# lswzjuer/pytorch-quantity

Hardware: AMD Instinct MI355X
Metric: calibration images/sec + int8-sim images/sec, ResNet-50 224², 1/2/4/8 GPU (higher is better)
Workload: dtype f32

## Files before the change

### pytorch-quantity_amd/csrc/fq_conv1x1_f32.hip

```cpp
#include "fq_common.h"
#include "fq_producer_stat.h"

#include <utility>

namespace fq {
namespace {

constexpr int kT = 256;
constexpr int kBK = 16;
constexpr int kStepWide = 8;
template <int WM> constexpr int step_of() { return WM == 2 ? kStepWide : kBK; }
typedef float f4v __attribute__((ext_vector_type(4)));
typedef float f16v __attribute__((ext_vector_type(16)));

struct C1Args {
    const float* x;
    const float* wt;
    const unsigned short* wsb;
    const float* bias;
    float* y;
    float* relu;
    const float* res;
    float* sum;
    int store_y;
// ... 1 lines not shown
    int Hin, R, S, pad;
    unsigned x_bytes, w_bytes, y_bytes;
    unsigned cols;
    unsigned tiles_m, tiles;
    int stream_stores;
    unsigned split_first, split_s, work;
    float* ws;
    unsigned* ws_count;
#ifdef FQ_C1_ABLATE
    int ablate;
#endif
};

#ifdef FQ_C1_ABLATE
#define FQ_C1_OFF(bit) (a.ablate & (bit))
#else
#define FQ_C1_OFF(bit) false
#endif

struct NoStat {
    __device__ __forceinline__ void add(float) {}
};

template <typename SC, typename SS, bool kStores>
struct AddStat {
    static constexpr bool kMayStore = kStores;
    SC c;
    SS s;
};
template <typename T> struct is_add_stat { static constexpr bool value = false; };
template <typename SC, typename SS, bool K> struct is_add_stat<AddStat<SC, SS, K>> { static constexpr bool value = true; };

template <int I>
struct Stage {
    static constexpr int value = I;
};

template <int WM, int WN, int BK = kBK>
struct Shape {
    static constexpr int BM = 64 * WM, BN = 64 * WN;
    static constexpr int kXRows = BK * BN / kT;
    static constexpr int kXStep = kT / BN > 0 ? kT / BN : 1;
    static constexpr int kWVecs = BK * BM / 4 / kT;
    static constexpr int kWRowStep = kT / (BM / 4);
    static constexpr int kFloats = 3 * BK * (BM + BN) + BM;
    static_assert(kXRows >= 1 && kWVecs >= 1 && BK % 4 == 0, "tile too small for 256 loading threads");
};

template <int WM, int WN, bool kRelu, bool kStream, bool kFullM, typename Stat>
__device__ __forceinline__ void c1_epilogue(const f16v (&acc)[WM][WN], const C1Args& a, Stat& stat, const float* s_bias,
                                            unsigned jbase, unsigned mbase, unsigned m0, unsigned n0, unsigned r, unsigned h) {
    const __amdgpu_buffer_rsrc_t yrs = __builtin_amdgcn_make_buffer_rsrc(a.y ? a.y : a.relu, 0, a.y ? a.y_bytes : 0u, 0x00020000);
    const __amdgpu_buffer_rsrc_t rrs = __builtin_amdgcn_make_buffer_rsrc(kRelu ? a.relu : a.y, 0, a.y_bytes, 0x00020000);
    constexpr int aux = kStream ? 2 : 0;
#pragma unroll
    for (int ni = 0; ni < WN; ++ni) {
        const unsigned jn = jbase + n0 + 32u * ni + r;
        if (jn < a.cols) {
            const unsigned n = jn / a.HWout, p = jn - n * a.HWout;
            const unsigned col4 = (n * a.Cout * a.HWout + p + (mbase + m0 + 4u * h) * a.HWout) * 4u;
#pragma unroll
            for (int mi = 0; mi < WM; ++mi) {
                f4v b4[4];
#pragma unroll
                for (int q = 0; q < 4; ++q) b4[q] = *reinterpret_cast<const f4v*>(s_bias + m0 + 32u * mi + 8u * q + 4u * h);
#pragma unroll
                for (int e = 0; e < 16; ++e) {
                    const unsigned dm = 32u * mi + (e & 3) + 8u * (e >> 2);
                    if (kFullM || mbase + m0 + 4u * h + dm < a.Cout) {
                        const float val = stat_map(stat, acc[mi][ni][e] + b4[e >> 2][e & 3]);
                        const int row4 = (int)(dm * a.HWout * 4u);
                        __builtin_amdgcn_raw_buffer_store_b32(__builtin_bit_cast(unsigned, val), yrs, (int)col4, row4, aux);
                        if (kRelu)
                            __builtin_amdgcn_raw_buffer_store_b32(__builtin_bit_cast(unsigned, relu_like_torch(val)), rrs, (int)col4,
                                                                  row4, aux);
                        stat.add(val);
                    }
                }
            }
        }
    }
}

template <int WM, int WN, bool kStoreY, bool kStoreSum, bool kStream, typename Stat>
__device__ __forceinline__ void c1_epilogue_add(const f16v (&acc)[WM][WN], const C1Args& a, Stat& stat, const float* s_bias,
                                                unsigned jbase, unsigned mbase, unsigned m0, unsigned n0, unsigned r, unsigned h) {
    const __amdgpu_buffer_rsrc_t yrs = __builtin_amdgcn_make_buffer_rsrc(kStoreY ? a.y : a.relu, 0, a.y_bytes, 0x00020000);
    const __amdgpu_buffer_rsrc_t srs = __builtin_amdgcn_make_buffer_rsrc(kStoreSum ? a.sum : a.relu, 0, a.y_bytes, 0x00020000);
    const __amdgpu_buffer_rsrc_t rrs = __builtin_amdgcn_make_buffer_rsrc(a.relu, 0, a.y_bytes, 0x00020000);
    const __amdgpu_buffer_rsrc_t ers = __builtin_amdgcn_make_buffer_rsrc(const_cast<float*>(a.res), 0, a.y_bytes, 0x00020000);
    constexpr int aux = kStream ? 2 : 0;
#pragma unroll
    for (int ni = 0; ni < WN; ++ni) {
        const unsigned jn = jbase + n0 + 32u * ni + r;
        if (jn < a.cols) {
            const unsigned n = jn / a.HWout, p = jn - n * a.HWout;
            const unsigned col4 = (n * a.Cout * a.HWout + p + (mbase + m0 + 4u * h) * a.HWout) * 4u;
#pragma unroll
            for (int mi = 0; mi < WM; ++mi) {
                float rv[16];
#pragma unroll
                for (int e = 0; e < 16; ++e) {
                    const unsigned dm = 32u * mi + (e & 3) + 8u * (e >> 2);
                    rv[e] = __builtin_bit_cast(float, __builtin_amdgcn_raw_buffer_load_b32(ers, (int)col4, (int)(dm * a.HWout * 4u), aux));
                }
                f4v b4[4];
#pragma unroll
                for (int q = 0; q < 4; ++q) b4[q] = *reinterpret_cast<const f4v*>(s_bias + m0 + 32u * mi + 8u * q + 4u * h);
#pragma unroll
                for (int e = 0; e < 16; ++e) {
                    const unsigned dm = 32u * mi + (e & 3) + 8u * (e >> 2);
                    const int row4 = (int)(dm * a.HWout * 4u);
                    const float val = acc[mi][ni][e] + b4[e >> 2][e & 3];
                    stat.c.add(val);
                    if (kStoreY) __builtin_amdgcn_raw_buffer_store_b32(__builtin_bit_cast(unsigned, val), yrs, (int)col4, row4, aux);
                    const float sm = val + rv[e];
                    stat.s.add(sm);
                    if (kStoreSum) __builtin_amdgcn_raw_buffer_store_b32(__builtin_bit_cast(unsigned, sm), srs, (int)col4, row4, aux);
                    __builtin_amdgcn_raw_buffer_store_b32(__builtin_bit_cast(unsigned, relu_like_torch(sm)), rrs, (int)col4, row4, aux);
                }
            }
        }
    }
}

template <int WM, int WN, typename Stat>
__device__ __forceinline__ void finish_tile(f16v (&acc)[WM][WN], const C1Args& a, Stat& stat, const float* s_bias, bool split, unsigned t,
                                            unsigned slice, unsigned jbase, unsigned mbase, unsigned m0, unsigned n0, unsigned r, unsigned h,
                                            unsigned tid, unsigned wave) {
    constexpr int BM = 64 * WM, BN = 64 * WN;
    bool finish = true;
    if (split) {
        const unsigned rr = t - a.split_first;
        constexpr unsigned kTileFloats = (unsigned)(BM * BN);
        float* const mine = a.ws + ((size_t)rr * a.split_s + slice) * kTileFloats;
#pragma unroll
        for (int mi = 0; mi < WM; ++mi)
#pragma unroll
            for (int ni = 0; ni < WN; ++ni)
#pragma unroll
                for (int q = 0; q < 4; ++q) {
                    const f4v v = {acc[mi][ni][4 * q], acc[mi][ni][4 * q + 1], acc[mi][ni][4 * q + 2], acc[mi][ni][4 * q + 3]};
                    *reinterpret_cast<f4v*>(mine + ((((mi * WN + ni) * 4 + q) * kT) + tid) * 4u) = v;
                }
        asm volatile("s_waitcnt vmcnt(0)" ::: "memory");
        __syncthreads();
        __shared__ unsigned s_last;
        if (tid == 0) {
            __builtin_amdgcn_fence(__ATOMIC_RELEASE, "agent");
            asm volatile("s_waitcnt vmcnt(0)" ::: "memory");
            const unsigned prev = __hip_atomic_fetch_add(a.ws_count + rr, 1u, __ATOMIC_RELAXED, __HIP_MEMORY_SCOPE_AGENT);
            const unsigned last = prev + 1u == a.split_s;
            if (last) {
                __builtin_amdgcn_fence(__ATOMIC_ACQUIRE, "agent");
                asm volatile("s_waitcnt vmcnt(0)" ::: "memory");
                __hip_atomic_store(a.ws_count + rr, 0u, __ATOMIC_RELAXED, __HIP_MEMORY_SCOPE_AGENT);
            }
            s_last = last;
        }
        __syncthreads();
        finish = s_last != 0u;
        if (finish) {
            if (wave != 0) {
                __builtin_amdgcn_fence(__ATOMIC_ACQUIRE, "agent");
                asm volatile("s_waitcnt vmcnt(0)" ::: "memory");
            }
#pragma unroll
            for (int mi = 0; mi < WM; ++mi)
#pragma unroll
                for (int ni = 0; ni < WN; ++ni)
#pragma unroll
                    for (int e = 0; e < 16; ++e) acc[mi][ni][e] = 0.0f;
            for (unsigned sl = 0; sl < a.split_s; ++sl) {
                const float* part = a.ws + ((size_t)rr * a.split_s + sl) * kTileFloats;
#pragma unroll
                for (int mi = 0; mi < WM; ++mi)
#pragma unroll
                    for (int ni = 0; ni < WN; ++ni)
#pragma unroll
                        for (int q = 0; q < 4; ++q) {
                            const f4v v = *reinterpret_cast<const f4v*>(part + ((((mi * WN + ni) * 4 + q) * kT) + tid) * 4u);
#pragma unroll
                            for (int c = 0; c < 4; ++c) acc[mi][ni][4 * q + c] += v[c];
                        }
            }
        }
    }
    if (finish) {
        const bool full_m = mbase + BM <= a.Cout;
#ifdef FQ_C1_ABLATE
        if (FQ_C1_OFF(1)) {
        } else
#endif
#define FQ_C1_EPI(R, S, F) c1_epilogue<WM, WN, R, S, F>(acc, a, stat, s_bias, jbase, mbase, m0, n0, r, h)
#define FQ_C1_ADD(Y, S, N) c1_epilogue_add<WM, WN, Y, S, N>(acc, a, stat, s_bias, jbase, mbase, m0, n0, r, h)
        if constexpr (is_add_stat<Stat>::value) {
            if constexpr (!Stat::kMayStore) {
                if (a.stream_stores) FQ_C1_ADD(false, false, true); else FQ_C1_ADD(false, false, false);
            } else
            if (a.stream_stores) {
                if (a.store_y) { if (a.sum) FQ_C1_ADD(true, true, true); else FQ_C1_ADD(true, false, true); }
                else { if (a.sum) FQ_C1_ADD(false, true, true); else FQ_C1_ADD(false, false, true); }
            } else {
                if (a.store_y) { if (a.sum) FQ_C1_ADD(true, true, false); else FQ_C1_ADD(true, false, false); }
                else { if (a.sum) FQ_C1_ADD(false, true, false); else FQ_C1_ADD(false, false, false); }
            }
// ... 661 lines not shown
    a.Cin = (unsigned)Cin; a.Cout = (unsigned)Cout; a.HWin = (unsigned)(Hin * Win); a.HWout = (unsigned)(Hout * Wout);
    a.Win = (unsigned)Win; a.Wout = (unsigned)Wout; a.stride = (unsigned)stride;
    a.Hin = Hin; a.R = R; a.S = S; a.pad = pad;
    a.cols = (unsigned)cols;
    a.x_bytes = (unsigned)(in_elems * 4);
    a.w_bytes = wsb ? (unsigned)(w_elems * 6) : (unsigned)(w_elems * 4);
    a.y_bytes = (unsigned)(out_elems * 4);
    a.tiles_m = a.tiles = 0;
    a.split_first = a.split_s = a.work = 0; a.ws = nullptr; a.ws_count = nullptr;
    a.stream_stores = out_elems * (relu_out && y ? 8 : 4) > ((size_t)256 << 20);
#ifdef FQ_C1_ABLATE
    a.ablate = env_int("FQ_C1_ABLATE", 0);
#endif
    hipStream_t st = as_stream(stream);
    static const int hist_per_cu = env_int("FQ_CONV1X1_HIST_WG_PER_CU", 0);
    static const int fast = [] { const char* e = getenv("FQ_HIST_IEEE_DIV"); return (e && e[0] && e[0] != '0') ? 0 : 1; }();
    const int mode = taps ? 2 : ((Cin % kBK) != 0 ? 1 : 0);
    static const int forced = env_int("FQ_CONV1X1_SHAPE", 0);
    const size_t tiles22 = ((cols + 127) / 128) * (size_t)((Cout + 127) / 128);
    const int shape = forced ? forced : ((Cout <= 64 || tiles22 <= (size_t)kCUs * 4) ? 12 : 22);
    if (wsb) {
        if (shape == 12) return launch_sb<1, 2>(a, max_inout, interval, hist_row, fast, qd, nullptr, nullptr, nullptr, nullptr, nullptr, nullptr, false, workspace, workspace_bytes, st);
        return launch_sb<2, 2>(a, max_inout, interval, hist_row, fast, qd, nullptr, nullptr, nullptr, nullptr, nullptr, nullptr, false, workspace, workspace_bytes, st);
    }
#define FQ_C1_LAUNCH(WM, WN)                                                                                       \
    do {                                                                                                           \
        if (mode == 2) launch<WM, WN, 2>(a, a.cols, max_inout, interval, hist_row, hist_per_cu, fast, qd, workspace, workspace_bytes, st);     \
        else if (mode == 1) launch<WM, WN, 1>(a, a.cols, max_inout, interval, hist_row, hist_per_cu, fast, qd, workspace, workspace_bytes, st); \
        else launch<WM, WN, 0>(a, a.cols, max_inout, interval, hist_row, hist_per_cu, fast, qd, workspace, workspace_bytes, st);               \
    } while (0)
    if (shape == 12) FQ_C1_LAUNCH(1, 2);
    else FQ_C1_LAUNCH(2, 2);
#undef FQ_C1_LAUNCH
    FQ_LAUNCH_CHECK();
    return FQ_OK;
}

}

extern "C" size_t fq_conv_f32_workspace_bytes(void) { return kSplitWsBytes; }

extern "C" int fq_conv1x1_f32(const float* x, const float* wt, const float* bias, float* y, float* relu_out, int N, int Cin,
                              int Hin, int Win, int Cout, int stride, float* max_inout, const float* interval,
                              int64_t* hist_row, void* workspace, size_t workspace_bytes, fq_stream_t stream) {
    return conv_f32_launch(x, wt, bias, y, relu_out, N, Cin, Hin, Win, Cout, 1, 1, stride, 0, max_inout, interval, hist_row,
                           workspace, workspace_bytes, stream);
}

extern "C" int fq_conv_kxk_f32(const float* x, const float* wt, const float* bias, float* y, float* relu_out, int N, int Cin,
                               int Hin, int Win, int Cout, int R, int S, int stride, int pad, float* max_inout,
                               const float* interval, int64_t* hist_row, void* workspace, size_t workspace_bytes,
                               fq_stream_t stream) {
    return conv_f32_launch(x, wt, bias, y, relu_out, N, Cin, Hin, Win, Cout, R, S, stride, pad, max_inout, interval, hist_row,
                           workspace, workspace_bytes, stream);
}

static int conv_add_launch(const float* x, const float* wt_in, const unsigned short* wsb, const float* bias, const float* res, float* y, float* sum,
                           float* relu_out, int N, int Cin, int Hin, int Win, int Cout, int stride, float* max_y, float* max_sum,
                           const float* interval_y, int64_t* hist_y, const float* interval_sum, int64_t* hist_sum,
                           void* workspace, size_t workspace_bytes, fq_stream_t stream) {
    const float* wt = wsb ? reinterpret_cast<const float*>(wsb) : wt_in;
    if (N < 0 || Cin <= 0 || Hin <= 0 || Win <= 0 || Cout <= 0 || stride < 1) return FQ_ERR_INVALID_ARG;
    if (N == 0) return FQ_OK;
    const bool hist = hist_y != nullptr;
    if (!x || !wt || !res || !relu_out) return FQ_ERR_INVALID_ARG;
    if (hist ? (!hist_sum || !interval_y || !interval_sum || hist_y == hist_sum) : (!max_y || !max_sum)) return FQ_ERR_INVALID_ARG;
    if ((Cin % kBK) != 0 || (Cout % 128) != 0 || (reinterpret_cast<uintptr_t>(wt) & 15u)) return FQ_ERR_UNSUPPORTED;
    const int Hout = (Hin - 1) / stride + 1, Wout = (Win - 1) / stride + 1;
    const size_t cols = (size_t)N * Hout * Wout;
    const size_t in_elems = (size_t)N * Cin * Hin * Win, out_elems = cols * Cout, w_elems = (size_t)Cin * Cout;
    if (cols >= 0xffffff00ULL || in_elems >= (1ULL << 30) || w_elems >= (1ULL << 30) || out_elems >= (1ULL << 30))
        return FQ_ERR_UNSUPPORTED;
    C1Args a;
    a.x = x; a.wt = wt; a.wsb = wsb; a.bias = bias; a.y = y; a.relu = relu_out; a.res = res; a.sum = sum; a.store_y = y != nullptr;
    a.Cin = (unsigned)Cin; a.Cout = (unsigned)Cout; a.HWin = (unsigned)(Hin * Win); a.HWout = (unsigned)(Hout * Wout);
    a.Win = (unsigned)Win; a.Wout = (unsigned)Wout; a.stride = (unsigned)stride;
    a.Hin = Hin; a.R = 1; a.S = 1; a.pad = 0;
    a.cols = (unsigned)cols;
    a.x_bytes = (unsigned)(in_elems * 4); a.w_bytes = wsb ? (unsigned)(w_elems * 6) : (unsigned)(w_elems * 4); a.y_bytes = (unsigned)(out_elems * 4);
    a.stream_stores = out_elems * (size_t)(8 + (y ? 4 : 0) + (sum ? 4 : 0)) > ((size_t)256 << 20) && (a.HWout % 16u) == 0;
    static const int stream_env = env_int("FQ_CONV_ADD_STREAM", -1);
    if (stream_env >= 0) a.stream_stores = stream_env;
#ifdef FQ_C1_ABLATE
    a.ablate = 0;
#endif
    static const int forced = env_int("FQ_CONV1X1_SHAPE", 0);
    const size_t tiles22 = ((cols + 127) / 128) * (size_t)(Cout / 128);
    const bool narrow = forced ? forced == 12 : tiles22 <= (size_t)kCUs * 4;
    hipStream_t st = as_stream(stream);
    a.tiles_m = (unsigned)Cout / (narrow ? 64u : 128u);
    a.tiles = (unsigned)((cols + 127) / 128) * a.tiles_m;
    if (wsb) {
        static const int fast_sb = [] { const char* e = getenv("FQ_HIST_IEEE_DIV"); return (e && e[0] && e[0] != '0') ? 0 : 1; }();
        if (narrow) return launch_sb<1, 2>(a, nullptr, nullptr, nullptr, fast_sb, nullptr, interval_y, hist_y, interval_sum, hist_sum, max_y, max_sum, true, workspace, workspace_bytes, st);
        return launch_sb<2, 2>(a, nullptr, nullptr, nullptr, fast_sb, nullptr, interval_y, hist_y, interval_sum, hist_sum, max_y, max_sum, true, workspace, workspace_bytes, st);
    }
    plan_split(a, (unsigned)Cin / (unsigned)(narrow ? step_of<1>() : step_of<2>()), workspace, workspace_bytes);
    if (hist) {
        static const int fast = [] { const char* e = getenv("FQ_HIST_IEEE_DIV"); return (e && e[0] && e[0] != '0') ? 0 : 1; }();
        static const int res12 = [] {
            int n = 0;
            if (hipOccupancyMaxActiveBlocksPerMultiprocessor(&n, conv1x1_f32_add_hist_kernel<1, 2>, kT, 0) != hipSuccess || n < 1) n = 1;
            return n;
        }();
        static const int res22 = [] {
            int n = 0;
            if (hipOccupancyMaxActiveBlocksPerMultiprocessor(&n, conv1x1_f32_add_hist_kernel<2, 2>, kT, 0) != hipSuccess || n < 1) n = 1;
            return n;
        }();
        unsigned grid = (unsigned)kCUs * (unsigned)(narrow ? res12 : res22);
        if (grid > a.work) grid = a.work;
        unsigned long long* hy = reinterpret_cast<unsigned long long*>(hist_y);
        unsigned long long* hs = reinterpret_cast<unsigned long long*>(hist_sum);
        if (narrow)
            hipLaunchKernelGGL((conv1x1_f32_add_hist_kernel<1, 2>), dim3(grid), dim3(kT), 0, st, a, interval_y, hy, interval_sum, hs, fast);
        else
            hipLaunchKernelGGL((conv1x1_f32_add_hist_kernel<2, 2>), dim3(grid), dim3(kT), 0, st, a, interval_y, hy, interval_sum, hs, fast);
    } else if (narrow) {
        hipLaunchKernelGGL((conv1x1_f32_add_absmax_kernel<1, 2>), dim3(a.work), dim3(kT), 0, st, a,
                           reinterpret_cast<unsigned int*>(max_y), reinterpret_cast<unsigned int*>(max_sum));
    } else {
        hipLaunchKernelGGL((conv1x1_f32_add_absmax_kernel<2, 2>), dim3(a.work), dim3(kT), 0, st, a,
                           reinterpret_cast<unsigned int*>(max_y), reinterpret_cast<unsigned int*>(max_sum));
    }
    FQ_LAUNCH_CHECK();
    return FQ_OK;
}

extern "C" int fq_conv1x1_add_f32(const float* x, const float* wt, const float* bias, const float* res, float* y, float* sum,
                                  float* relu_out, int N, int Cin, int Hin, int Win, int Cout, int stride, float* max_y,
                                  float* max_sum, void* workspace, size_t workspace_bytes, fq_stream_t stream) {
    return conv_add_launch(x, wt, nullptr, bias, res, y, sum, relu_out, N, Cin, Hin, Win, Cout, stride, max_y, max_sum, nullptr, nullptr,
                           nullptr, nullptr, workspace, workspace_bytes, stream);
}

extern "C" int fq_conv1x1_add_hist_f32(const float* x, const float* wt, const float* bias, const float* res, float* relu_out,
                                       int N, int Cin, int Hin, int Win, int Cout, int stride, const float* interval_y,
                                       int64_t* hist_y, const float* interval_sum, int64_t* hist_sum, void* workspace,
                                       size_t workspace_bytes, fq_stream_t stream) {
    if (!hist_y) return FQ_ERR_INVALID_ARG;
    return conv_add_launch(x, wt, nullptr, bias, res, nullptr, nullptr, relu_out, N, Cin, Hin, Win, Cout, stride, nullptr, nullptr, interval_y,
                           hist_y, interval_sum, hist_sum, workspace, workspace_bytes, stream);
}

static bool qd_params(int bit, int bitwidth, QdStat* qd) {
    if ((bitwidth != 8 && bitwidth != 16) || bit < -120 || bit > 120) return false;
    qd->scale = ldexpf(1.0f, bit); qd->inv = ldexpf(1.0f, -bit);
    qd->lo = bitwidth == 8 ? -128.0f : -32768.0f; qd->hi = bitwidth == 8 ? 127.0f : 32767.0f;
    return true;
}

extern "C" int fq_conv1x1_qd_f32(const float* x, const float* wt, const float* bias, float* y, int N, int Cin, int Hin, int Win,
                                 int Cout, int stride, int bit, int bitwidth, void* workspace, size_t workspace_bytes,
                                 fq_stream_t stream) {
    QdStat qd;
    if (!qd_params(bit, bitwidth, &qd)) return FQ_ERR_INVALID_ARG;
    return conv_f32_launch(x, wt, bias, y, nullptr, N, Cin, Hin, Win, Cout, 1, 1, stride, 0, nullptr, nullptr, nullptr, workspace,
                           workspace_bytes, stream, &qd);
}

extern "C" int fq_conv_kxk_qd_f32(const float* x, const float* wt, const float* bias, float* y, int N, int Cin, int Hin, int Win,
                                  int Cout, int R, int S, int stride, int pad, int bit, int bitwidth, void* workspace,
                                  size_t workspace_bytes, fq_stream_t stream) {
    QdStat qd;
    if (!qd_params(bit, bitwidth, &qd)) return FQ_ERR_INVALID_ARG;
    return conv_f32_launch(x, wt, bias, y, nullptr, N, Cin, Hin, Win, Cout, R, S, stride, pad, nullptr, nullptr, nullptr, workspace,
                           workspace_bytes, stream, &qd);
// ... 50 lines not shown
```

### pytorch-quantity_amd/csrc/fq_conv_wino_f32.hip

```cpp
#include "fq_common.h"
#include "fq_producer_stat.h"

#ifndef FQ_WINO_ABLATE
#define FQ_WINO_ABLATE 0
#endif
#define FQ_WINO_OFF(bit) ((FQ_WINO_ABLATE) & (bit))

namespace fq {
namespace {

constexpr unsigned kBK = 64;
constexpr unsigned kCS = 8;
template <int WT>
struct Geo {
    static constexpr int kT = 256 * WT;
    static constexpr unsigned kWaves = 4u * WT;
    static constexpr unsigned kBT = 32u * WT;
    static constexpr unsigned kKkBytes = kBT * 16u;
    static constexpr unsigned kPlane = 2u * kKkBytes;
    static constexpr unsigned kStageBytes = 16u * kPlane;
    static constexpr unsigned kLdsBytes = 3u * kStageBytes;
};
constexpr unsigned kOob = 0x80000000u;
typedef float f2v __attribute__((ext_vector_type(2)));
typedef float f4v __attribute__((ext_vector_type(4)));
typedef float f16v __attribute__((ext_vector_type(16)));
typedef unsigned u2v __attribute__((__vector_size__(2 * sizeof(unsigned))));

struct WArgs {
    const float* x;
    const float* u;
    const float* bias;
    float* y;
    float* relu;
    unsigned Cin, Cout, H, W, HW, TH, TW, tiles_img, tiles, tiles_t, work;
    unsigned x_bytes, u_bytes, y_bytes;
    int stream_stores;
};

struct NoStat {
    __device__ __forceinline__ void add(float) {}
};

__device__ __forceinline__ void stat_add_if(NoStat&, bool, float) {}
__device__ __forceinline__ void stat_add_if(QdStat&, bool, float) {}
__device__ __forceinline__ void stat_add_if(MaxStat& s, bool ok, float v) { s.add(ok ? v : 0.0f); }
template <bool kFast>
__device__ __forceinline__ void stat_add_if(HistStat<kFast>& s, bool ok, float v) { if (ok) s.add(v); }

template <int WT, bool kEven, bool kRelu, bool kStream, typename Stat>
__device__ __forceinline__ void wino_epilogue(const f16v (&acc)[8], unsigned ph, unsigned wave, unsigned lane, char* smem, const WArgs& a,
                                              Stat& stat, unsigned kbase, unsigned tbase, unsigned r, unsigned h) {
    const __amdgpu_buffer_rsrc_t yrs = __builtin_amdgcn_make_buffer_rsrc(a.y ? a.y : a.relu, 0, a.y ? a.y_bytes : 0u, 0x00020000);
    const __amdgpu_buffer_rsrc_t rrs = __builtin_amdgcn_make_buffer_rsrc(kRelu ? a.relu : a.y, 0, a.y_bytes, 0x00020000);
    constexpr int aux = kStream ? 2 : 0;
    const unsigned t = tbase + r;
    const bool tile_ok = t < a.tiles;
    const unsigned tc = tile_ok ? t : 0u;
    const unsigned n = tc / a.tiles_img, rem = tc - n * a.tiles_img, ty = rem / a.TW, tx = rem - ty * a.TW;
    const unsigned oy = 2u * ty + ph, ox = 2u * tx;
    const bool row_ok = tile_ok && (kEven || oy < a.H), px1_ok = row_ok && (kEven || ox + 1u < a.W);
    const unsigned off0 = (((n * a.Cout + kbase + 4u * h) * a.H + oy) * a.W + ox) * 4u;
    const unsigned v0 = row_ok ? off0 : kOob, v1 = px1_ok ? off0 + 4u : kOob;
    f4v b4[4];
#pragma unroll
    for (int q = 0; q < 4; ++q)
        b4[q] = a.bias ? *reinterpret_cast<const f4v*>(a.bias + kbase + 8u * q + 4u * h) : f4v{0.f, 0.f, 0.f, 0.f};
    constexpr unsigned kSlot = Geo<WT>::kWaves * 64u;
    f2v* const mine = reinterpret_cast<f2v*>(smem) + wave * 64u + lane;
    const f2v* const theirs = reinterpret_cast<const f2v*>(smem) + (wave ^ (2u * WT)) * 64u + lane;
    float na[16][2], nb[16][2];
    __syncthreads();
#pragma unroll
    for (int e = 0; e < 16; ++e) {
        float lo[4], hi[4];
#pragma unroll
        for (int c = 0; c < 4; ++c) {
            asm volatile("v_accvgpr_read_b32 %0, %1" : "=v"(lo[c]) : "a"(acc[c][e]));
            asm volatile("v_accvgpr_read_b32 %0, %1" : "=v"(hi[c]) : "a"(acc[4 + c][e]));
        }
        na[e][0] = (lo[0] + lo[1]) + lo[2]; na[e][1] = (lo[1] - lo[2]) - lo[3];
        nb[e][0] = (hi[0] + hi[1]) + hi[2]; nb[e][1] = (hi[1] - hi[2]) - hi[3];
        mine[e * kSlot] = ph == 0 ? f2v{nb[e][0], nb[e][1]} : f2v{na[e][0], na[e][1]};
        __builtin_amdgcn_sched_barrier(0);
    }
    __syncthreads();
#pragma unroll
    for (int e = 0; e < 16; ++e) {
        const unsigned dm = (e & 3) + 8u * (e >> 2);
        const int row4 = (int)(dm * a.HW * 4u);
        const f2v got = theirs[e * kSlot];
        float tc4[2];
#pragma unroll
        for (int c = 0; c < 2; ++c)
            tc4[c] = ph == 0 ? (na[e][c] + nb[e][c]) + got[c] : (got[c] - na[e][c]) - nb[e][c];
        const float bias = b4[e >> 2][e & 3];
        float o0 = tc4[0] + bias, o1 = tc4[1] + bias;
        o0 = stat_map(stat, o0); o1 = stat_map(stat, o1);
        if (kEven) {
            __builtin_amdgcn_raw_buffer_store_b64(__builtin_bit_cast(u2v, f2v{o0, o1}), yrs, (int)v0, row4, aux);
            if (kRelu)
                __builtin_amdgcn_raw_buffer_store_b64(__builtin_bit_cast(u2v, f2v{relu_like_torch(o0), relu_like_torch(o1)}), rrs, (int)v0, row4, aux);
        } else {
            __builtin_amdgcn_raw_buffer_store_b32(__builtin_bit_cast(unsigned, o0), yrs, (int)v0, row4, aux);
            __builtin_amdgcn_raw_buffer_store_b32(__builtin_bit_cast(unsigned, o1), yrs, (int)v1, row4, aux);
            if (kRelu) {
                __builtin_amdgcn_raw_buffer_store_b32(__builtin_bit_cast(unsigned, relu_like_torch(o0)), rrs, (int)v0, row4, aux);
                __builtin_amdgcn_raw_buffer_store_b32(__builtin_bit_cast(unsigned, relu_like_torch(o1)), rrs, (int)v1, row4, aux);
            }
        }
        stat_add_if(stat, row_ok, o0);
        stat_add_if(stat, px1_ok, o1);
        __builtin_amdgcn_sched_barrier(0);
    }
}

struct TileIn {
    unsigned xo[4];
    bool c0ok, c2ok, c3ok, shift1;
    int endrow;
};

template <int WT>
__device__ __forceinline__ TileIn tile_in(const WArgs& a, unsigned tb, unsigned lane) {
    TileIn t;
    const unsigned ti = tb * Geo<WT>::kBT + (WT == 1 ? lane & 31u : lane);
    const bool tile_ok = ti < a.tiles;
    const unsigned tc = tile_ok ? ti : 0u;
    const unsigned n = tc / a.tiles_img, rem = tc - n * a.tiles_img, ty = rem / a.TW, tx = rem - ty * a.TW;
    const int iy0 = (int)(2u * ty) - 1;
    const unsigned nb = n * a.Cin * a.HW;
    t.c0ok = tx != 0u; t.c2ok = 2u * tx + 1u < a.W; t.c3ok = 2u * tx + 2u < a.W;
    t.shift1 = tile_ok && tc == 0u;
    const bool last_col = tile_ok && tc + a.tiles_img >= a.tiles && tx + 1u == a.TW;
    t.endrow = -1;
#pragma unroll
    for (int i = 0; i < 4; ++i) {
        const int iy = iy0 + i;
        const bool ok = tile_ok && (unsigned)iy < a.H;
        const bool end = last_col && (unsigned)iy + 1u == a.H;
        t.xo[i] = ok ? (end ? nb + a.HW - 4u : nb + (unsigned)iy * a.W + 2u * tx - 1u) * 4u : kOob;
        t.endrow = end ? i : t.endrow;
    }
    if (t.shift1) t.xo[1] = 0u;
    const unsigned second = WT == 1 ? (lane >> 5) * a.HW * 4u : 0u;
#pragma unroll
    for (int i = 0; i < 4; ++i) t.xo[i] += second;
    return t;
}

template <int WT, bool kOddW, typename Stat>
__device__ __forceinline__ void wino_tiles(const WArgs& a, Stat& stat, char* smem) {
    typedef Geo<WT> G_;
    constexpr unsigned kBT = G_::kBT, kKkBytes = G_::kKkBytes, kPlane = G_::kPlane, kStageBytes = G_::kStageBytes;
    const unsigned tid = threadIdx.x, lane = tid & 63u;
    const unsigned wave = (unsigned)__builtin_amdgcn_readfirstlane((int)(tid >> 6));
    const unsigned r = lane & 31u, h = lane >> 5;
    const unsigned wk = WT == 2 ? (wave & 3u) >> 1 : wave & 1u, wt = WT == 2 ? wave & 1u : 0u, ph = wave / (2u * WT);
    const unsigned tkk = WT == 2 ? wave & 1u : h, tks = WT == 2 ? wave >> 1 : wave, ttile = WT == 2 ? lane : r;
    const unsigned tch = WT == 2 ? wave : 2u * wave;
    const __amdgpu_buffer_rsrc_t xrs = __builtin_amdgcn_make_buffer_rsrc(const_cast<float*>(a.x), 0, a.x_bytes, 0x00020000);
    const __amdgpu_buffer_rsrc_t urs = __builtin_amdgcn_make_buffer_rsrc(const_cast<float*>(a.u), 0, a.u_bytes, 0x00020000);
    const unsigned vrd = h * kKkBytes + (wt * 32u + r) * 16u + ph * 8u * kPlane;
    const unsigned vwr = tkk * kKkBytes + ttile * 16u + tks * 4u;
    const unsigned nsteps = a.Cin / kCS;
    const unsigned upos = 2u * a.Cout * 16u;
    const unsigned uvo = (h * a.Cout + wk * 32u + r) * 16u;
    const unsigned G = gridDim.x, G8 = G & ~7u, g = blockIdx.x;
    const unsigned v0 = g < G8 ? (g & 7u) * (G8 >> 3) + (g >> 3) : g;

    for (unsigned wi = v0; wi < a.work; wi += G) {
        const unsigned kb = wi / a.tiles_t, tb = wi - kb * a.tiles_t;
        const TileIn ti = tile_in<WT>(a, tb, lane);
        const bool ends = (tb + 1u) * kBT + a.TW >= a.tiles;
        f4v d[4];
        auto xload = [&](unsigned s) {
            const int so = (int)((s * kCS + tch) * a.HW * 4u);
#pragma unroll
            for (int i = 0; i < 4; ++i) d[i] = __builtin_bit_cast(f4v, __builtin_amdgcn_raw_buffer_load_b128(xrs, (int)ti.xo[i], so, 0));
        };
        auto transform_store = [&](unsigned stage_off) {
            if (tb == 0u) d[1] = ti.shift1 ? f4v{0.0f, d[1][0], d[1][1], d[1][2]} : d[1];
            if (ends) {
#pragma unroll
                for (int i = 0; i < 4; ++i) {
                    const f4v sh = kOddW ? f4v{d[i][2], d[i][3], 0.0f, 0.0f} : f4v{d[i][1], d[i][2], d[i][3], 0.0f};
                    d[i] = ti.endrow == i ? sh : d[i];
                }
            }
#pragma unroll
            for (int i = 0; i < 4; ++i) {
                d[i][0] = ti.c0ok ? d[i][0] : 0.0f;
                d[i][3] = ti.c3ok ? d[i][3] : 0.0f;
            }
            if (kOddW) {
#pragma unroll
                for (int i = 0; i < 4; ++i) d[i][2] = ti.c2ok ? d[i][2] : 0.0f;
            }
            const f4v t0 = d[0] - d[2], t1 = d[1] + d[2], t2 = d[2] - d[1], t3 = d[1] - d[3];
            const f4v t[4] = {t0, t1, t2, t3};
            char* const w = smem + stage_off + vwr;
#pragma unroll
            for (int i = 0; i < 4; ++i) {
                *reinterpret_cast<float*>(w + (unsigned)(4 * i) * kPlane) = t[i][0] - t[i][2];
                *reinterpret_cast<float*>(w + (unsigned)(4 * i + 1) * kPlane) = t[i][1] + t[i][2];
                *reinterpret_cast<float*>(w + (unsigned)(4 * i + 2) * kPlane) = t[i][2] - t[i][1];
                *reinterpret_cast<float*>(w + (unsigned)(4 * i + 3) * kPlane) = t[i][1] - t[i][3];
            }
        };
        f4v ua[8];
        auto uload = [&](int e, unsigned s) {
            ua[e] = __builtin_bit_cast(f4v, __builtin_amdgcn_raw_buffer_load_b128(
                urs, (int)uvo, (int)((s * 16u + 8u * ph + (unsigned)e) * upos + kb * (kBK * 16u)), 0));
        };
        f4v bq[2][4];
        auto bload = [&](int half, unsigned stage_off, int e0) {
#pragma unroll
            for (int e = 0; e < 4; ++e) bq[half][e] = *reinterpret_cast<const f4v*>(smem + stage_off + vrd + (unsigned)(e0 + e) * kPlane);
        };
        f16v acc[8];
#pragma unroll
        for (int e = 0; e < 8; ++e)
#pragma unroll
            for (int i = 0; i < 16; ++i) acc[e][i] = 0.0f;
        auto mfma_half = [&](int half, int e0, unsigned sn) {
#pragma unroll
            for (int k = 0; k < 4; ++k)
#pragma unroll
                for (int e = 0; e < 4; ++e) {
                    if (!FQ_WINO_OFF(16)) acc[e0 + e] = __builtin_amdgcn_mfma_f32_32x32x2f32(ua[e0 + e][k], bq[half][e][k], acc[e0 + e], 0, 0, 0);
                    else acc[e0 + e][k] += ua[e0 + e][k] * bq[half][e][k];
                }
            if (!FQ_WINO_OFF(2)) {
#pragma unroll
                for (int e = 0; e < 4; ++e) uload(e0 + e, sn);
            }
        };

        xload(0);
        transform_store(0u);
        xload(nsteps > 1 ? 1u : 0u);
#pragma unroll
        for (int e = 0; e < 8; ++e) uload(e, 0);
        __syncthreads();
        bload(0, 0u, 0);
        if (FQ_WINO_OFF(64)) bload(1, 0u, 4);
        unsigned cur = 0;
        for (unsigned s = 0; s < nsteps; ++s) {
            const unsigned nxt = cur == 2u * kStageBytes ? 0u : cur + kStageBytes;
            const unsigned sn = s + 1 < nsteps ? s + 1 : s;
            if (!FQ_WINO_OFF(64)) bload(1, cur, 4);
            mfma_half(0, 0, sn);
            if (!FQ_WINO_OFF(4)) transform_store(nxt);
            if (!FQ_WINO_OFF(1)) xload(s + 2 < nsteps ? s + 2 : s);
            if (!FQ_WINO_OFF(32)) __syncthreads();
            if (!FQ_WINO_OFF(64)) bload(0, nxt, 0);
            mfma_half(1, 4, sn);
            cur = nxt;
        }
        const unsigned kbase = kb * kBK + wk * 32u, tbase = tb * kBT + wt * 32u;
        asm volatile("s_nop 15\n\ts_nop 15" ::: "memory");
        const bool even = ((a.H | a.W) & 1u) == 0u;
#define FQ_WINO_EPI(E, R, S) wino_epilogue<WT, E, R, S>(acc, ph, wave, lane, smem, a, stat, kbase, tbase, r, h)
        if (FQ_WINO_OFF(8)) {
            float sum = 0.0f;
#pragma unroll
            for (int e = 0; e < 8; ++e)
#pragma unroll
                for (int i = 0; i < 16; ++i) sum += acc[e][i];
            if (sum == 12345.678f) a.y[0] = sum;
        } else if (even) {
            if (a.relu) { if (a.stream_stores) FQ_WINO_EPI(true, true, true); else FQ_WINO_EPI(true, true, false); }
            else { if (a.stream_stores) FQ_WINO_EPI(true, false, true); else FQ_WINO_EPI(true, false, false); }
        } else {
            if (a.relu) FQ_WINO_EPI(false, true, false); else FQ_WINO_EPI(false, false, false);
        }
#undef FQ_WINO_EPI
        __syncthreads();
    }
}

#define FQ_WINO_TILES(ST) do { if (a.W & 1u) wino_tiles<WT, true>(a, ST, wino_smem); else wino_tiles<WT, false>(a, ST, wino_smem); } while (0)

template <int WT>
__global__ __launch_bounds__(Geo<WT>::kT) __attribute__((amdgpu_waves_per_eu(2, 2))) void wino_f32_kernel(const WArgs a) {
    extern __shared__ __attribute__((aligned(16))) char wino_smem[];
    NoStat st;
    FQ_WINO_TILES(st);
}

template <int WT>
__global__ __launch_bounds__(Geo<WT>::kT) __attribute__((amdgpu_waves_per_eu(2, 2))) void wino_f32_absmax_kernel(const WArgs a, unsigned int* __restrict__ max_bits) {
    extern __shared__ __attribute__((aligned(16))) char wino_smem[];
    MaxStat st;
    FQ_WINO_TILES(st);
    publish_max<Geo<WT>::kT>(st.m, max_bits);
}

template <int WT>
__global__ __launch_bounds__(Geo<WT>::kT) __attribute__((amdgpu_waves_per_eu(2, 2))) void wino_f32_qd_kernel(const WArgs a, const QdStat qd) {
    extern __shared__ __attribute__((aligned(16))) char wino_smem[];
    QdStat st = qd;
    FQ_WINO_TILES(st);
}

template <int WT>
__global__ __launch_bounds__(Geo<WT>::kT) __attribute__((amdgpu_waves_per_eu(2, 2))) void wino_f32_hist_kernel(
    const WArgs a, const float* __restrict__ interval, unsigned long long* __restrict__ hist_row, const int allow_fast) {
    extern __shared__ __attribute__((aligned(16))) char wino_smem[];
    __shared__ unsigned int s_bins[FQ_BINS + kWave];
    for (int b = threadIdx.x; b < FQ_BINS + kWave; b += Geo<WT>::kT) s_bins[b] = 0u;
    __syncthreads();
    const float iv = *interval;
    unsigned int* park = s_bins + FQ_BINS + (threadIdx.x & (kWave - 1));
    if (allow_fast && fast_quotient_ok(iv)) {
        HistStat<true> st{s_bins, park, iv, 1.0f / iv};
        FQ_WINO_TILES(st);
    } else {
        HistStat<false> st{s_bins, park, iv, 1.0f / iv};
        FQ_WINO_TILES(st);
    }
    hist_flush<Geo<WT>::kT>(s_bins, hist_row);
}
#undef FQ_WINO_TILES

__global__ __launch_bounds__(256) void wino_pack_kernel(const float* __restrict__ w, float* __restrict__ u, unsigned Cin, unsigned Cout) {
    const unsigned i = blockIdx.x * 256u + threadIdx.x;
    if (i >= Cin * Cout) return;
    const unsigned k = i / Cin, c = i - k * Cin;
    const float* g = w + (size_t)i * 9u;
    double gg[3][3], t[4][3];
    for (int a = 0; a < 3; ++a)
        for (int b = 0; b < 3; ++b) gg[a][b] = (double)g[3 * a + b];
    for (int b = 0; b < 3; ++b) {
        t[0][b] = gg[0][b];
        t[1][b] = 0.5 * (gg[0][b] + gg[1][b] + gg[2][b]);
        t[2][b] = 0.5 * (gg[0][b] - gg[1][b] + gg[2][b]);
        t[3][b] = gg[2][b];
    }
    const unsigned cb = c / kCS, kk = c & 1u, ks = (c % kCS) >> 1;
    for (int a = 0; a < 4; ++a) {
        const double o[4] = {t[a][0], 0.5 * (t[a][0] + t[a][1] + t[a][2]), 0.5 * (t[a][0] - t[a][1] + t[a][2]), t[a][2]};
        for (int b = 0; b < 4; ++b) {
            const unsigned e = 4u * (unsigned)a + (unsigned)b;
            u[((((size_t)cb * 16u + e) * 2u + kk) * Cout + k) * 4u + ks] = (float)o[b];
        }
    }
}

bool wino_shape_ok(int N, int Cin, int Hin, int Win, int Cout) {
    if (N < 0 || Cin <= 0 || Hin <= 0 || Win <= 0 || Cout <= 0) return false;
    if ((Cin % (int)kCS) != 0 || (Cout % (int)kBK) != 0) return false;
    if ((size_t)Hin * Win < 4) return false;
    const size_t in_bytes = (size_t)N * Cin * Hin * Win * 4, out_bytes = (size_t)N * Cout * Hin * Win * 4;
    const size_t tiles = (size_t)N * ((Hin + 1) / 2) * ((Win + 1) / 2);
    const size_t work = ((tiles + 31) / 32) * (size_t)(Cout / (int)kBK);
    return in_bytes < (1ULL << 31) && out_bytes < (1ULL << 31) && (size_t)Cin * Cout * 64 < (1ULL << 31) && tiles < (1ULL << 30) &&
           work < (1ULL << 31);
}

}
// ... 84 lines not shown
```

Before: 8773.

## Software-pipeline conv epilogues: prefetch residual and next-tile input during stores

The 1x1 conv residual-add epilogue now loads residual values one quad-block ahead, interleaving them with stores, and gets a full-N fast path without per-column bounds checks. The Winograd kernel stages bias through shared memory and issues the next work item's first input load inside the current epilogue, so the load latency hides behind the output stores. It also hoists transform_store for the next tile to the end of the loop. The cost is more register pressure, inline asm with hand-set waitcnt counts, and more complex control flow that could be fragile.

```diff
diff --git a/pytorch-quantity_amd/csrc/fq_conv1x1_f32.hip b/pytorch-quantity_amd/csrc/fq_conv1x1_f32.hip
--- a/pytorch-quantity_amd/csrc/fq_conv1x1_f32.hip
+++ b/pytorch-quantity_amd/csrc/fq_conv1x1_f32.hip
@@ -107,46 +107,78 @@
     }
 }
 
-template <int WM, int WN, bool kStoreY, bool kStoreSum, bool kStream, typename Stat>
-__device__ __forceinline__ void c1_epilogue_add(const f16v (&acc)[WM][WN], const C1Args& a, Stat& stat, const float* s_bias,
-                                                unsigned jbase, unsigned mbase, unsigned m0, unsigned n0, unsigned r, unsigned h) {
+template <int WM, int WN, bool kStoreY, bool kStoreSum, bool kStream, bool kFullN, typename Stat>
+__device__ __forceinline__ void c1_epilogue_add_blocks(const f16v (&acc)[WM][WN], const C1Args& a, Stat& stat, const float* s_bias,
+                                                       unsigned jbase, unsigned mbase, unsigned m0, unsigned n0, unsigned r, unsigned h) {
     const __amdgpu_buffer_rsrc_t yrs = __builtin_amdgcn_make_buffer_rsrc(kStoreY ? a.y : a.relu, 0, a.y_bytes, 0x00020000);
     const __amdgpu_buffer_rsrc_t srs = __builtin_amdgcn_make_buffer_rsrc(kStoreSum ? a.sum : a.relu, 0, a.y_bytes, 0x00020000);
     const __amdgpu_buffer_rsrc_t rrs = __builtin_amdgcn_make_buffer_rsrc(a.relu, 0, a.y_bytes, 0x00020000);
     const __amdgpu_buffer_rsrc_t ers = __builtin_amdgcn_make_buffer_rsrc(const_cast<float*>(a.res), 0, a.y_bytes, 0x00020000);
     constexpr int aux = kStream ? 2 : 0;
+    constexpr int kBlocks = WM * WN;
+    bool ok[WN];
+    unsigned col4[WN];
 #pragma unroll
     for (int ni = 0; ni < WN; ++ni) {
         const unsigned jn = jbase + n0 + 32u * ni + r;
-        if (jn < a.cols) {
-            const unsigned n = jn / a.HWout, p = jn - n * a.HWout;
-            const unsigned col4 = (n * a.Cout * a.HWout + p + (mbase + m0 + 4u * h) * a.HWout) * 4u;
-#pragma unroll
-            for (int mi = 0; mi < WM; ++mi) {
-                float rv[16];
-#pragma unroll
-                for (int e = 0; e < 16; ++e) {
-                    const unsigned dm = 32u * mi + (e & 3) + 8u * (e >> 2);
-                    rv[e] = __builtin_bit_cast(float, __builtin_amdgcn_raw_buffer_load_b32(ers, (int)col4, (int)(dm * a.HWout * 4u), aux));
-                }
-                f4v b4[4];
-#pragma unroll
-                for (int q = 0; q < 4; ++q) b4[q] = *reinterpret_cast<const f4v*>(s_bias + m0 + 32u * mi + 8u * q + 4u * h);
-#pragma unroll
-                for (int e = 0; e < 16; ++e) {
-                    const unsigned dm = 32u * mi + (e & 3) + 8u * (e >> 2);
-                    const int row4 = (int)(dm * a.HWout * 4u);
-                    const float val = acc[mi][ni][e] + b4[e >> 2][e & 3];
-                    stat.c.add(val);
-                    if (kStoreY) __builtin_amdgcn_raw_buffer_store_b32(__builtin_bit_cast(unsigned, val), yrs, (int)col4, row4, aux);
-                    const float sm = val + rv[e];
-                    stat.s.add(sm);
-                    if (kStoreSum) __builtin_amdgcn_raw_buffer_store_b32(__builtin_bit_cast(unsigned, sm), srs, (int)col4, row4, aux);
-                    __builtin_amdgcn_raw_buffer_store_b32(__builtin_bit_cast(unsigned, relu_like_torch(sm)), rrs, (int)col4, row4, aux);
-                }
-            }
-        }
-    }
+        ok[ni] = kFullN || jn < a.cols;
+        const unsigned jc = kFullN ? jn : min(jn, a.cols - 1u);
+        const unsigned n = jc / a.HWout, p = jc - n * a.HWout;
+        col4[ni] = (n * a.Cout * a.HWout + p + (mbase + m0 + 4u * h) * a.HWout) * 4u;
+    }
+    float rv[16];
+    auto qload = [&](int b, int q) {
+#ifdef FQ_C1_ABLATE
+        if (a.ablate & 8) {
+#pragma unroll
+            for (int c = 0; c < 4; ++c) rv[4 * q + c] = 1.0f;
+            return;
+        }
+#endif
+#pragma unroll
+        for (int c = 0; c < 4; ++c) {
+            const unsigned dm = 32u * (b % WM) + c + 8u * q;
+            rv[4 * q + c] = __builtin_bit_cast(float, __builtin_amdgcn_raw_buffer_load_b32(ers, (int)col4[b / WM], (int)(dm * a.HWout * 4u), aux));
+        }
+    };
+#pragma unroll
+    for (int q = 0; q < 4; ++q) qload(0, q);
+    __builtin_amdgcn_sched_barrier(0);
+    auto bias_quad = [&](int g) { return *reinterpret_cast<const f4v*>(s_bias + m0 + 32u * ((g >> 2) % WM) + 8u * (g & 3) + 4u * h); };
+    f4v b4[2];
+    b4[0] = bias_quad(0);
+#pragma unroll
+    for (int g = 0; g < 4 * kBlocks; ++g) {
+        const int b = g >> 2, q = g & 3, ni = b / WM, mi = b % WM;
+        if (g + 1 < 4 * kBlocks) b4[(g + 1) & 1] = bias_quad(g + 1);
+        if (ok[ni]) {
+#pragma unroll
+            for (int c = 0; c < 4; ++c) {
+                const int e = 4 * q + c;
+                const unsigned dm = 32u * mi + c + 8u * q;
+                const int row4 = (int)(dm * a.HWout * 4u);
+                const float val = acc[mi][ni][e] + b4[g & 1][c];
+                stat.c.add(val);
+                if (kStoreY) __builtin_amdgcn_raw_buffer_store_b32(__builtin_bit_cast(unsigned, val), yrs, (int)col4[ni], row4, aux);
+                const float sm = val + rv[e];
+                stat.s.add(sm);
+                if (kStoreSum) __builtin_amdgcn_raw_buffer_store_b32(__builtin_bit_cast(unsigned, sm), srs, (int)col4[ni], row4, aux);
+                __builtin_amdgcn_raw_buffer_store_b32(__builtin_bit_cast(unsigned, relu_like_torch(sm)), rrs, (int)col4[ni], row4, aux);
+            }
+        }
+        __builtin_amdgcn_sched_barrier(0);
+        if (b + 1 < kBlocks) qload(b + 1, q);
+        __builtin_amdgcn_sched_barrier(0);
+    }
+}
+
+template <int WM, int WN, bool kStoreY, bool kStoreSum, bool kStream, typename Stat>
+__device__ __forceinline__ void c1_epilogue_add(const f16v (&acc)[WM][WN], const C1Args& a, Stat& stat, const float* s_bias,
+                                                unsigned jbase, unsigned mbase, unsigned m0, unsigned n0, unsigned r, unsigned h) {
+    if (jbase + 64u * WN <= a.cols)
+        c1_epilogue_add_blocks<WM, WN, kStoreY, kStoreSum, kStream, true>(acc, a, stat, s_bias, jbase, mbase, m0, n0, r, h);
+    else
+        c1_epilogue_add_blocks<WM, WN, kStoreY, kStoreSum, kStream, false>(acc, a, stat, s_bias, jbase, mbase, m0, n0, r, h);
 }
 
 template <int WM, int WN, typename Stat>
@@ -974,7 +1006,7 @@
     static const int stream_env = env_int("FQ_CONV_ADD_STREAM", -1);
     if (stream_env >= 0) a.stream_stores = stream_env;
 #ifdef FQ_C1_ABLATE
-    a.ablate = 0;
+    a.ablate = env_int("FQ_C1_ABLATE", 0);
 #endif
     static const int forced = env_int("FQ_CONV1X1_SHAPE", 0);
     const size_t tiles22 = ((cols + 127) / 128) * (size_t)(Cout / 128);
diff --git a/pytorch-quantity_amd/csrc/fq_conv_wino_f32.hip b/pytorch-quantity_amd/csrc/fq_conv_wino_f32.hip
--- a/pytorch-quantity_amd/csrc/fq_conv_wino_f32.hip
+++ b/pytorch-quantity_amd/csrc/fq_conv_wino_f32.hip
@@ -26,6 +26,7 @@
 typedef float f4v __attribute__((ext_vector_type(4)));
 typedef float f16v __attribute__((ext_vector_type(16)));
 typedef unsigned u2v __attribute__((__vector_size__(2 * sizeof(unsigned))));
+typedef unsigned u4v __attribute__((ext_vector_type(4)));
 
 struct WArgs {
     const float* x;
@@ -47,10 +48,13 @@
 __device__ __forceinline__ void stat_add_if(MaxStat& s, bool ok, float v) { s.add(ok ? v : 0.0f); }
 template <bool kFast>
 __device__ __forceinline__ void stat_add_if(HistStat<kFast>& s, bool ok, float v) { if (ok) s.add(v); }
-
-template <int WT, bool kEven, bool kRelu, bool kStream, typename Stat>
+template <typename T> struct is_hist_stat { static constexpr bool value = false; };
+template <bool kFast> struct is_hist_stat<HistStat<kFast>> { static constexpr bool value = true; };
+
+template <int WT, bool kEven, bool kRelu, bool kStream, typename Stat, typename Prefetch>
 __device__ __forceinline__ void wino_epilogue(const f16v (&acc)[8], unsigned ph, unsigned wave, unsigned lane, char* smem, const WArgs& a,
-                                              Stat& stat, unsigned kbase, unsigned tbase, unsigned r, unsigned h) {
+                                              Stat& stat, unsigned kbase, unsigned tbase, unsigned r, unsigned h, float bias64, unsigned wk,
+                                              Prefetch& prefetch) {
     const __amdgpu_buffer_rsrc_t yrs = __builtin_amdgcn_make_buffer_rsrc(a.y ? a.y : a.relu, 0, a.y ? a.y_bytes : 0u, 0x00020000);
     const __amdgpu_buffer_rsrc_t rrs = __builtin_amdgcn_make_buffer_rsrc(kRelu ? a.relu : a.y, 0, a.y_bytes, 0x00020000);
     constexpr int aux = kStream ? 2 : 0;
@@ -62,15 +66,13 @@
     const bool row_ok = tile_ok && (kEven || oy < a.H), px1_ok = row_ok && (kEven || ox + 1u < a.W);
     const unsigned off0 = (((n * a.Cout + kbase + 4u * h) * a.H + oy) * a.W + ox) * 4u;
     const unsigned v0 = row_ok ? off0 : kOob, v1 = px1_ok ? off0 + 4u : kOob;
-    f4v b4[4];
-#pragma unroll
-    for (int q = 0; q < 4; ++q)
-        b4[q] = a.bias ? *reinterpret_cast<const f4v*>(a.bias + kbase + 8u * q + 4u * h) : f4v{0.f, 0.f, 0.f, 0.f};
+    float* const s_bias = reinterpret_cast<float*>(smem + 2u * Geo<WT>::kStageBytes);
     constexpr unsigned kSlot = Geo<WT>::kWaves * 64u;
     f2v* const mine = reinterpret_cast<f2v*>(smem) + wave * 64u + lane;
     const f2v* const theirs = reinterpret_cast<const f2v*>(smem) + (wave ^ (2u * WT)) * 64u + lane;
     float na[16][2], nb[16][2];
     __syncthreads();
+    if (threadIdx.x < 64u) s_bias[threadIdx.x] = bias64;
 #pragma unroll
     for (int e = 0; e < 16; ++e) {
         float lo[4], hi[4];
@@ -85,16 +87,19 @@
         __builtin_amdgcn_sched_barrier(0);
     }
     __syncthreads();
+    prefetch();
+    f4v b4 = {0.f, 0.f, 0.f, 0.f};
 #pragma unroll
     for (int e = 0; e < 16; ++e) {
         const unsigned dm = (e & 3) + 8u * (e >> 2);
         const int row4 = (int)(dm * a.HW * 4u);
         const f2v got = theirs[e * kSlot];
+        if ((e & 3) == 0) b4 = *reinterpret_cast<const f4v*>(s_bias + wk * 32u + 8u * (unsigned)(e >> 2) + 4u * h);
         float tc4[2];
 #pragma unroll
         for (int c = 0; c < 2; ++c)
             tc4[c] = ph == 0 ? (na[e][c] + nb[e][c]) + got[c] : (got[c] - na[e][c]) - nb[e][c];
-        const float bias = b4[e >> 2][e & 3];
+        const float bias = b4[e & 3];
         float o0 = tc4[0] + bias, o1 = tc4[1] + bias;
         o0 = stat_map(stat, o0); o1 = stat_map(stat, o1);
         if (kEven) {
@@ -113,6 +118,8 @@
         stat_add_if(stat, px1_ok, o1);
         __builtin_amdgcn_sched_barrier(0);
     }
+    constexpr int kStores = (kEven ? 16 : 32) * (kRelu ? 2 : 1);
+    asm volatile("s_waitcnt vmcnt(%0)" ::"n"(kStores > 63 ? 63 : kStores) : "memory");
 }
 
 struct TileIn {
@@ -169,11 +176,29 @@
     const unsigned G = gridDim.x, G8 = G & ~7u, g = blockIdx.x;
     const unsigned v0 = g < G8 ? (g & 7u) * (G8 >> 3) + (g >> 3) : g;
 
+    constexpr bool kAhead = !is_hist_stat<Stat>::value && !FQ_WINO_OFF(128);
+    f4v d[4];
+    TileIn ti;
+    unsigned kb = 0, tb = 0;
+    bool ends = false;
+    auto item = [&](unsigned wi) {
+        kb = wi / a.tiles_t; tb = wi - kb * a.tiles_t;
+        ti = tile_in<WT>(a, tb, lane);
+        ends = (tb + 1u) * kBT + a.TW >= a.tiles;
+    };
+    const u4v xrs_words = {(unsigned)(reinterpret_cast<uintptr_t>(a.x) & 0xffffffffu), (unsigned)(reinterpret_cast<uintptr_t>(a.x) >> 32) & 0xffffu,
+                           a.x_bytes, 0x00020000u};
+    auto xload0_hidden = [&](const TileIn& t) {
+        const unsigned so = tch * a.HW * 4u;
+#pragma unroll
+        for (int i = 0; i < 4; ++i)
+            asm volatile("s_nop 4\n\tbuffer_load_dwordx4 %0, %1, %2, %3 offen" : "=&v"(d[i]) : "v"(t.xo[i]), "s"(xrs_words), "s"(so) : "memory");
+    };
+    auto x_prefetch_take = [&]() {
+        asm volatile("" : "+v"(d[0]), "+v"(d[1]), "+v"(d[2]), "+v"(d[3]));
+    };
+    if (v0 < a.work) item(v0);
     for (unsigned wi = v0; wi < a.work; wi += G) {
-        const unsigned kb = wi / a.tiles_t, tb = wi - kb * a.tiles_t;
-        const TileIn ti = tile_in<WT>(a, tb, lane);
-        const bool ends = (tb + 1u) * kBT + a.TW >= a.tiles;
-        f4v d[4];
         auto xload = [&](unsigned s) {
             const int so = (int)((s * kCS + tch) * a.HW * 4u);
 #pragma unroll
@@ -237,8 +262,11 @@
             }
         };
 
-        xload(0);
-        transform_store(0u);
+        const float bias64 = (a.bias && tid < 64u) ? a.bias[kb * kBK + tid] : 0.0f;
+        if (wi == v0) {
+            xload(0);
+            transform_store(0u);
+        }
         xload(nsteps > 1 ? 1u : 0u);
 #pragma unroll
         for (int e = 0; e < 8; ++e) uload(e, 0);
@@ -259,9 +287,11 @@
             cur = nxt;
         }
         const unsigned kbase = kb * kBK + wk * 32u, tbase = tb * kBT + wt * 32u;
+        const bool more = wi + G < a.work;
+        auto prefetch = [&]() { if (kAhead && more) xload0_hidden(tile_in<WT>(a, (wi + G) % a.tiles_t, lane)); };
         asm volatile("s_nop 15\n\ts_nop 15" ::: "memory");
         const bool even = ((a.H | a.W) & 1u) == 0u;
-#define FQ_WINO_EPI(E, R, S) wino_epilogue<WT, E, R, S>(acc, ph, wave, lane, smem, a, stat, kbase, tbase, r, h)
+#define FQ_WINO_EPI(E, R, S) wino_epilogue<WT, E, R, S>(acc, ph, wave, lane, smem, a, stat, kbase, tbase, r, h, bias64, wk, prefetch)
         if (FQ_WINO_OFF(8)) {
             float sum = 0.0f;
 #pragma unroll
@@ -277,6 +307,15 @@
         }
 #undef FQ_WINO_EPI
         __syncthreads();
+        if (more) {
+            item(wi + G);
+            if (!kAhead) {
+                xload0_hidden(ti);
+                asm volatile("s_waitcnt vmcnt(0)" ::: "memory");
+            }
+            x_prefetch_take();
+            transform_store(0u);
+        }
     }
 }
 
```

Measured after the change: 8710. No clear change (-0.7%).
